# nilsfriess/MultigridMC

Hardware: AMD Instinct MI355X
Metric: MGMC V-cycle samples/sec + fine-smoother HBM GB/s, 512³ lattice, 1/2/4/8 GPUs (higher is better)
Workload: dtype f64

## Files before the change

### multigridmc_amd/csrc/mgmc_capi.hip

```cpp
#include "mgmc_internal.hpp"

namespace mgmc_host {
std::mutex g_err_mutex;
std::string g_last_error;
std::atomic<int> g_live_handles{0};
void set_global_error(const std::string& s) {
    std::lock_guard<std::mutex> lock(g_err_mutex);
    g_last_error = s;
}
}

namespace {
constexpr int LDS_POISON_DOUBLES = 80 * 1024 / 8;
__global__ void __launch_bounds__(1024) k_lds_poison() {
    extern __shared__ double lds[];
    const double nan = __builtin_nan("");
    for (int q = threadIdx.x; q < LDS_POISON_DOUBLES; q += blockDim.x) lds[q] = nan;
    __syncthreads();
    if (lds[(threadIdx.x * 7) % LDS_POISON_DOUBLES] == 0.0) asm volatile("" ::: "memory");
}
__global__ void __launch_bounds__(256) k_poison_interior(Layout L, double* __restrict__ x) {
    const int i = blockIdx.x * blockDim.x + threadIdx.x + 1;
    const int j = blockIdx.y + 1;
    const int k = L.dim == 3 ? (int)blockIdx.z + 1 : 0;
// ... 91 lines not shown
    }
    const int dim = lv.spec.dim, np = lv.spec.npoints;
#define DISPATCH(D, P)                                                       \
    if (dim == D && np == P) {                                               \
        if (noise)                                                           \
            launch_sweep_t<D, P, true>(lv, x, f, g, direction, s);           \
        else                                                                 \
            launch_sweep_t<D, P, false>(lv, x, f, g, direction, s);          \
        return;                                                              \
    }
    DISPATCH(3, 7) DISPATCH(3, 27) DISPATCH(2, 5) DISPATCH(2, 9)
#undef DISPATCH
}

template <int XP, int TY, int NT, int MINW = 1>
void launch_zsweep_t(const Level& lv, ZSweepArgs a, bool prolong, hipStream_t s, int nch) {
    a.ntx = (lv.L.nx / 2) / XP;
    a.nty = (lv.L.ny - 1 + TY - 1) / TY;
    a.ntz = (lv.L.nz - 1 + a.tz - 1) / a.tz;
    const int ntiles = a.ntx * a.nty * (a.zpairs ? (a.ntz + 1) / 2 * 2 : a.ntz);
    const int nb = (ntiles + 7) / 8 * 8;
    const size_t lds = zsweep_lds_bytes(XP, TY, prolong);
    int ex;
    const bool pow2 = std::isnormal(a.alpha) && std::frexp(std::fabs(a.alpha), &ex) == 0.5 && ex > -900 && ex < 900;
    const dim3 grid(nb, 1, nch);
    const bool lrf = a.lr.e != nullptr;
    if (prolong && pow2 && lrf)
        hipLaunchKernelGGL((k_zsweep_rb7<XP, TY, NT, 2, MINW, true>), grid, dim3(NT), lds, s, a);
    else if (prolong && pow2)
        hipLaunchKernelGGL((k_zsweep_rb7<XP, TY, NT, 2, MINW>), grid, dim3(NT), lds, s, a);
    else if (prolong && lrf)
        hipLaunchKernelGGL((k_zsweep_rb7<XP, TY, NT, 1, MINW, true>), grid, dim3(NT), lds, s, a);
    else if (prolong)
        hipLaunchKernelGGL((k_zsweep_rb7<XP, TY, NT, 1, MINW>), grid, dim3(NT), lds, s, a);
    else if (lrf)
        hipLaunchKernelGGL((k_zsweep_rb7<XP, TY, NT, 0, MINW, true>), grid, dim3(NT), lds, s, a);
    else
        hipLaunchKernelGGL((k_zsweep_rb7<XP, TY, NT, 0, MINW>), grid, dim3(NT), lds, s, a);
}

static int zsweep_depth(const Level& lv, int ty, int tzmax) {
// ... 3 lines not shown
    return tz;
}

static int zsweep_plain_rows(const Level& lv, int nch) {
    const int tz = zsweep_depth(lv, ZS_TY, ZS_TZ);
    auto ntiles = [&](int ty) {
        const long long nz = (lv.L.nz - 1 + tz - 1) / tz;
        return (long long)((lv.L.nx / 2) / ZS_XP) * ((lv.L.ny - 1 + ty - 1) / ty) * ((nz + 1) / 2 * 2) * nch;
    };
    const long long slots = 2LL * lv.num_cu;
    return (ZS_TYP != ZS_TY && ZS_NTP == ZS_NT && ntiles(ZS_TY) < slots && ntiles(ZS_TYP) <= slots) ? ZS_TYP : ZS_TY;
}

void launch_zsweep(const Level& lv, const double* xin, double* xout, const double* f, const GibbsArg& g0,
                   int direction, const Level* coarse, const double* xc, double alpha, hipStream_t s, int nch = 1,
                   const LRRhsArg* lr = nullptr) {
    ZSweepArgs a;
    a.lr = lr ? *lr : LRRhsArg{nullptr};
    a.cs = lv.L.nstore;
    a.csc = coarse ? coarse->L.nstore : 0;
    a.L = lv.L;
    a.xin = xin;
    a.xout = xout;
    a.f = f;
    a.xc = xc;
    a.Lc = coarse ? coarse->L : lv.L;
    a.alpha = alpha;
    a.S = lv.S;
    a.G = g0;
    a.G.colour = (direction == MGMC_FORWARD) ? 0 : 1;
    a.zpairs = 0;
    if (coarse) {
        a.tz = zsweep_depth(lv, ZS_TYP, ZS_TZP);
        launch_zsweep_t<ZS_XP, ZS_TYP, ZS_NTP, ZS_MINWP>(lv, a, true, s, nch);
        return;
    }
    a.tz = zsweep_depth(lv, ZS_TY, ZS_TZ);
    a.zpairs = 1;
    if (zsweep_plain_rows(lv, nch) != ZS_TY) {
        launch_zsweep_t<ZS_XP, ZS_TYP, ZS_NTP, ZS_MINWP>(lv, a, false, s, nch);
        return;
    }
    launch_zsweep_t<ZS_XP, ZS_TY, ZS_NT, ZS_MINW>(lv, a, false, s, nch);
}

bool pairs_eligible(const LevelSpec& sp, const Layout& L) {
    return (sp.npoints == 27 || sp.npoints == 9) && L.nx / 2 >= 1 && L.nx / 2 <= 256 && L.nx % 2 == 0;
}

bool quads_eligible(const LevelSpec& sp, const Layout& L, uint32_t paths) {
    if (!pairs_eligible(sp, L) || (paths & PATH_NO_QUADS)) return false;
    return sp.dim == 2 || L.nx / 2 <= tune::QUADS_MAXPAIR;
}

void launch_rb2d(const Level& lv, const double* xin, double* xout, const double* f, const GibbsArg& g, int direction,
                 bool noise, hipStream_t s, int nch = 1) {
    const int ntx = (lv.L.nx - 1 + RB2_TW - 1) / RB2_TW, nty = (lv.L.ny - 1 + RB2_TH - 1) / RB2_TH;
    const int c1 = direction == MGMC_FORWARD ? 0 : 1;
// ... 191 lines not shown
        else if (pre)                                                                                              \
            hipLaunchKernelGGL((k_coarse_ssor_lds<D, P, true>), grid, block, lds, s, lv.L, lv.x, lv.f, lv.S, g,   \
                               nsweeps, nc, chs, nullptr, 0);                                                      \
        else                                                                                                       \
            hipLaunchKernelGGL((k_coarse_ssor_lds<D, P, false>), grid, block, lds, s, lv.L, lv.x, lv.f, lv.S, g,  \
                               nsweeps, nc, chs, nullptr, 0);                                                      \
    } while (0)
    if (dim == 3 && np == 27) MGMC_COARSE_LAUNCH(3, 27);
    else if (dim == 3 && np == 7) MGMC_COARSE_LAUNCH(3, 7);
    else if (dim == 2 && np == 9) MGMC_COARSE_LAUNCH(2, 9);
    else MGMC_COARSE_LAUNCH(2, 5);
#undef MGMC_COARSE_LAUNCH
}


template <int NPTS, int CX, int CY, int NT, bool SYM = false, bool LRF = false>
void launch_zresrestrict_t(const Level& lf, const Level& lc, const double* x, const double* f, double* fc, double* xc,
                           hipStream_t s, int nch, const TailNoiseLaunch* tn = nullptr, const LRRhsArg* lr = nullptr,
                           const PreNoiseLaunch* pn = nullptr) {
    ZRestrictArgs a;
    memset(&a, 0, sizeof(a));
    if (LRF) a.lr = *lr;
    if (pn) {
        a.pn = pn->job;
        a.key = pn->key;
        a.sample = pn->sample;
    }
    a.csf = lf.L.nstore;
    a.csc = lc.L.nstore;
    a.Lf = lf.L;
    a.Lc = lc.L;
// ... 18 lines not shown
        const long long slots = per_cu * lf.num_cu;
        const long long per_chunk = (long long)a.ntx * a.nty;
        long long best = -1;
        for (int kz = 2; kz <= 16; ++kz) {
            const long long tiles = per_chunk * ((lc.L.nz - 1 + kz - 1) / kz);
            const long long cost = ((tiles + slots - 1) / slots) * (2 * kz + 2);
            if (best < 0 || cost < best) {
                best = cost;
                a.kz = kz;
            }
        }
    }
    a.ntz = (lc.L.nz - 1 + a.kz - 1) / a.kz;
    const int nt = a.ntx * a.nty * a.ntz;
    const int nb = (nt + 7) / 8 * 8;
    if (tn && !LRF) {
        a.nblk_main = nb;
        a.jobs = tn->jobs;
        a.njobs = tn->njobs;
        a.zb = tn->zb;
        a.zbs = tn->zbs;
        a.key = tn->key;
        a.chain0 = tn->chain0;
        a.seed_hi = tn->seed_hi;
        a.sample = tn->sample;
        const int nextra = (int)std::min<long long>((tn->zbs + NT - 1) / NT, 64);
        hipLaunchKernelGGL((k_zresrestrict<NPTS, CX, CY, NT, true, SYM>), dim3(nb + nextra, 1, nch), dim3(NT),
                           zrestrict_lds_bytes(CX, CY), s, a);
        return;
    }
    hipLaunchKernelGGL((k_zresrestrict<NPTS, CX, CY, NT, false, SYM, LRF>), dim3(nb, 1, nch), dim3(NT),
                       zrestrict_lds_bytes(CX, CY), s, a);
}

bool zres_lrf_capable(const Level& lf, const Level& lc) {
    return lf.spec.dim == 3 && lf.spec.npoints == 7 && !lf.field && !(lf.paths & PATH_NO_ZRESTRICT) &&
           lc.L.nx >= 8 && lc.L.nx >= tune::ZR_SMALL_NX;
}

bool zres_draws_noise(const Level& lf, const Level& lc) {
    return lf.spec.dim == 3 && lf.spec.npoints == 27 && !lf.field && !(lf.paths & PATH_NO_ZRESTRICT) &&
           lc.L.nx >= tune::ZR_SMALL_NX;
}

void launch_residual_restrict(const Level& lf, const Level& lc, const double* x, const double* f, double* fc,
                              double* xc, int zero_xc, hipStream_t s, int nch, const TailNoiseLaunch* tn,
                              bool skip_xc, const LRRhsArg* lr, const PreNoiseLaunch* pn) {
    const bool zr = lf.spec.dim == 3 && zero_xc && !lf.field && !(lf.paths & PATH_NO_ZRESTRICT) && lc.L.nx >= 8;
    if (nch > 1 && !zr) {
        for (int c = 0; c < nch; ++c)
            launch_residual_restrict(lf, lc, chain_ptr(x, lf, c), chain_ptr(f, lf, c), chain_ptr(fc, lc, c),
                                     chain_ptr(xc, lc, c), zero_xc, s, 1);
        return;
    }
    if (lf.field) {
        dim3 block(64, 4, 1);
        dim3 grid = grid3(lf.L.nx - 1, lf.L.ny - 1, lf.spec.dim == 3 ? lf.L.nz - 1 : 1, block);
        dim3 gc = grid3(lc.L.nx - 1, lc.L.ny - 1, lf.spec.dim == 3 ? lc.L.nz - 1 : 1, block);
        if (lf.spec.dim == 3) {
            hipLaunchKernelGGL((k_fresidual<3>), grid, block, 0, s, lf.L, x, f, lf.F, lf.rbuf);
            hipLaunchKernelGGL((k_restrict<3>), gc, block, 0, s, lf.L, lc.L, (const double*)lf.rbuf, fc);
        } else {
            hipLaunchKernelGGL((k_fresidual<2>), grid, block, 0, s, lf.L, x, f, lf.F, lf.rbuf);
            hipLaunchKernelGGL((k_restrict<2>), gc, block, 0, s, lf.L, lc.L, (const double*)lf.rbuf, fc);
        }
        if (zero_xc) hipMemsetAsync(xc, 0, lc.L.nstore * sizeof(double), s);
        return;
    }
    if (lf.spec.dim == 3 && zero_xc && !(lf.paths & PATH_NO_ZRESTRICT) && lc.L.nx >= 8) {
        const bool small = lc.L.nx < tune::ZR_SMALL_NX;
        if (skip_xc) xc = nullptr;
        if (lr) {
            if ((long long)((lc.L.nx + 62) / 64) * ((lc.L.ny + 6) / 8) * (lc.L.nz - 1) >= tune::ZR7_WIDE_MIN_TILES)
                launch_zresrestrict_t<7, 64, 8, 512, false, true>(lf, lc, x, f, fc, xc, s, nch, nullptr, lr);
            else launch_zresrestrict_t<7, 64, 4, 256, false, true>(lf, lc, x, f, fc, xc, s, nch, nullptr, lr);
        } else if (lf.spec.npoints == 7) {
            if (small) launch_zresrestrict_t<7, 16, 4, 64>(lf, lc, x, f, fc, xc, s, nch, tn);
            else if ((long long)((lc.L.nx + 62) / 64) * ((lc.L.ny + 6) / 8) * (lc.L.nz - 1) >= tune::ZR7_WIDE_MIN_TILES)
                launch_zresrestrict_t<7, 64, 8, 512>(lf, lc, x, f, fc, xc, s, nch);
            else launch_zresrestrict_t<7, 64, 4, 256>(lf, lc, x, f, fc, xc, s, nch);
        } else {
            if (small && lf.fold) launch_zresrestrict_t<27, 16, 4, 64, true>(lf, lc, x, f, fc, xc, s, nch, tn);
            else if (small) launch_zresrestrict_t<27, 16, 4, 64>(lf, lc, x, f, fc, xc, s, nch, tn);
            else if (lf.fold)
                launch_zresrestrict_t<27, tune::ZR27_CX, tune::ZR27_CY, 256, true>(lf, lc, x, f, fc, xc, s, nch, nullptr,
                                                                                   nullptr, pn);
            else launch_zresrestrict_t<27, 64, 4, 256>(lf, lc, x, f, fc, xc, s, nch, nullptr, nullptr, pn);
        }
        return;
    }
// ... 835 lines not shown
        Op& rr = h->ops[q];
        Op& sw = h->ops[q + 1];
        if (rr.kind != OP_RESIDUAL_RESTRICT || sw.kind != OP_SWEEP || sw.level != rr.level + 1 || sw.src != 0 ||
            rr.zpre != 0)
            continue;
        const Level& lf = h->levels[rr.level];
        const Level& lc = h->levels[sw.level];
        const bool zr = lf.spec.dim == 3 && !lf.field && !(lf.paths & PATH_NO_ZRESTRICT) && lc.L.nx >= 8;
        const bool quads3 = lc.quads && lc.spec.dim == 3;
        if (!zr || !(lc.jsweep || quads3) || lc.field) continue;
        rr.xzero = 1;
        sw.xzero = 1;
    }
}

constexpr long long PN_MAX_PAIRS = 2LL << 20;

int plan_drawn_noise(mgmc_handle* h) {
    for (Op& op : h->ops) {
        op.pnz = nullptr;
        op.pn_dst = nullptr;
        op.pn_tag = 0;
    }
    if ((h->paths & PATH_NO_POST_NOISE) || h->nchains != 1) return MGMC_OK;
    std::vector<double2*> buf(h->levels.size(), nullptr);
    auto level_buf = [&](int l) -> double2* {
        if (!buf[l]) {
            const Level& lv = h->levels[l];
            const long long n = (long long)(lv.L.nx / 2) * (lv.L.ny - 1) * (lv.L.nz - 1);
            if (hipMalloc(&buf[l], (size_t)n * sizeof(double2)) != hipSuccess) {
// ... 51 lines not shown
            continue;
        }
        TailArgs* d = h->tail_args[ti];
        const int npn = (int)jobs.size();
        HIPCHK(h, hipMemcpy(d->pn, jobs.data(), jobs.size() * sizeof(PostNoiseJob), hipMemcpyHostToDevice));
        HIPCHK(h, hipMemcpy(&d->npn, &npn, sizeof(int), hipMemcpyHostToDevice));
        h->tail_pn_wg[ti] = tune::TAIL_PN_WG > 0 ? tune::TAIL_PN_WG : std::max(1, h->levels[0].num_cu - h->nchains);
    }
    return MGMC_OK;
}

int build_tails(mgmc_handle* h) {
    int rc = build_tails_only(h);
    if (rc == MGMC_OK) fuse_sweep_restrict(h);
    if (rc == MGMC_OK) mark_zero_inputs(h);
    if (rc == MGMC_OK) rc = plan_drawn_noise(h);
    return rc;
}

void enqueue_ops(mgmc_handle* h, size_t begin, size_t end, hipStream_t s) {
    const uint64_t* sample = h->ctrl;
    const int nch = h->nchains;
    for (size_t q = begin; q < end; ++q) {
        const Op& op = h->ops[q];
        Level& lv = h->levels[op.level];
        if (h->poison)
            hipLaunchKernelGGL(k_lds_poison, dim3(8 * lv.num_cu), dim3(1024), LDS_POISON_DOUBLES * sizeof(double), s);
        switch (op.kind) {
            case OP_SWEEP: {
                GibbsArg g = make_gibbs(h, lv, op.tag, 0, sample);
                const bool lr = lv.lr.m > 0;
                double* fs = lv.f;
                LRRhsArg lrr{nullptr};
                const bool inplace = lr && lv.lr.rhs_inplace;
                if (lr && !op.lr_skip_patch)
                    fs = lr_rhs(h, lv, LR_PATCH_NOISE, lv.f, op.tag, sample, s, nch, -1, inplace ? &lrr : nullptr);
                else if (inplace)
                    lrr = LRRhsArg{lv.lr.rhs_e + nch};
                else if (lr && lv.lr.dense_path)
                    fs = lv.lr.fe2;
                double* xo = lv.x;
                if (lv.zsweep) {
                    const Level* lc = op.prolong ? &h->levels[op.level + 1] : nullptr;
                    xo = lv.buf(1 - op.src);
                    launch_zsweep(lv, lv.buf(op.src), xo, fs, g, op.direction, lc, lc ? lc->x : nullptr,
                                  h->cfg.coarse_scaling, s, nch, lrr.e ? &lrr : nullptr);
                } else if (lv.quads) {
                    xo = lv.buf(1 - op.src);
                    launch_quads(lv, lv.buf(op.src), xo, fs, g, op.direction, s, nch, op.xzero != 0, op.pnz);
                } else if (lv.rb2d) {
                    xo = lv.buf(1 - op.src);
                    launch_rb2d(lv, lv.buf(op.src), xo, fs, g, op.direction, true, s, nch);
                } else if (lv.pairs) {
                    launch_pairs(lv, lv.x, fs, g, op.direction, s, nch);
                } else {
                    launch_sweep(lv, lv.x, fs, g, op.direction, true, s, nch);
                }
                if (lr && lv.lr.small)
                    lr_small(h, lv, xo, op.direction, op.lr_next, op.lr_next_tag, sample, s, nch);
                else if (lr)
                    lr_fix(lv, xo, op.direction, lv.lr.dense_path && !inplace ? nullptr : lv.f, s, nch);
// ... 34 lines not shown
                                lv.lr.rhs_inplace && op.zpre == 0 ? &lrr : nullptr);
                }
                if (op.zpre > 0) {
                    const int ti = op.zpre - 1;
                    const TailNoiseLaunch tn{h->tail_jobs[ti], h->tail_njobs[ti], h->tail_zb[ti], h->tail_zn[ti],
                                             h->key, (uint32_t)h->chain, (uint32_t)(h->seed >> 32), sample};
                    launch_residual_restrict(lv, lc, lv.buf(op.src), fr, lc.f, lc.x, 1, s, nch, &tn);
                } else {
                    PreNoiseLaunch pnl;
                    if (op.pn_dst) {
                        pnl.job = PostNoiseJob{lc.L.nx, lc.L.ny, lc.L.nz, op.pn_tag, op.pn_dst};
                        pnl.key = h->key;
                        pnl.sample = sample;
                    }
                    launch_residual_restrict(lv, lc, lv.buf(op.src), fr, lc.f, lc.x, 1, s, nch, nullptr, op.xzero != 0,
                                             lrr.e ? &lrr : nullptr, op.pn_dst ? &pnl : nullptr);
                    if (op.xzero && h->poison)
                        for (int c = 0; c < nch; ++c)
                            hipLaunchKernelGGL(k_poison_interior, dim3((lc.L.nx - 1 + 255) / 256, lc.L.ny - 1,
                                                                       lc.spec.dim == 3 ? lc.L.nz - 1 : 1),
                                               dim3(256), 0, s, lc.L, chain_ptr(lc.x, lc, c));
                }
                if (lr && lv.lr.dense_path && !lrr.e)
                    ;
                else if (lr && (op.lr_post_patch || op.lr_coarse_patch))
                    lr_restore_patch(h, op, lv, lc, sample, s, nch);
                else if (lr)
                    lr_restore(lv, lv.f, s, nch, lrr.e != nullptr);
                break;
            }
            case OP_PROLONGATE: {
// ... 746 lines not shown

        } else res = "k_residual_restrict<" + std::to_string(dim) + "," + std::to_string(np) + ">";
    }
    std::string text = "sweep=" + sweep;
    if (!post.empty()) text += ";post_sweep=" + post;
    bool by_rr = false, by_tail = false;
    for (size_t q = 0; q < h->ops.size(); ++q) {
        const Op& op = h->ops[q];
        if (op.kind != OP_SWEEP || op.level != level || !op.pnz) continue;
        if (q > 0 && h->ops[q - 1].kind == OP_RESIDUAL_RESTRICT && h->ops[q - 1].pn_dst == op.pnz) by_rr = true;
        else by_tail = true;
    }
    if (by_rr || by_tail)
        text += std::string(";noise=") + (by_rr && by_tail ? "restriction+tail" : by_rr ? "restriction" : "tail");
    if (!res.empty()) text += ";residual_restrict=" + res;
    if (lv.lr.m > 0)
        text += std::string(";lowrank=") + (lv.lr.rhs_inplace ? "dense,rhs_inplace" : lv.lr.dense_path ? "dense"
                                             : lv.lr.small ? "small" : "rows");
    snprintf(out, n, "%s", text.c_str());
    return MGMC_OK;
}

static int put_fine(mgmc_handle* h, double* v, int c, const double* host, size_t n, const char* what) {
    if (!h || !host) return fail(h, MGMC_E_INVALID, "null argument");
    if (n != h->levels[0].spec.ndof) return fail(h, MGMC_E_INVALID, std::string(what) + " size mismatch");
    if (c >= h->nchains) return fail(h, MGMC_E_INVALID, "chain index out of range");
    HIPCHK(h, hipSetDevice(h->device));
    const size_t ns = h->levels[0].L.nstore;
    int rc = upload(h, 0, host, v + (size_t)std::max(c, 0) * ns);
    if (rc) return rc;
    if (c < 0)
        for (int q = 1; q < h->nchains; ++q)
            HIPCHK(h, hipMemcpyAsync(v + q * ns, v, ns * sizeof(double), hipMemcpyDeviceToDevice, h->stream));
    return MGMC_OK;
}

int mgmc_set_rhs(mgmc_handle* h, const double* f, size_t n) {
    int rc = put_fine(h, h ? h->levels[0].f : nullptr, -1, f, n, "rhs");
    if (rc) return rc;
    HIPCHK(h, hipStreamSynchronize(h->stream));
    return MGMC_OK;
}

static int set_state_impl(mgmc_handle* h, int c, const double* x, size_t n) {
    int rc = put_fine(h, h ? h->levels[0].x : nullptr, c, x, n, "state");
    if (rc) return rc;
    HIPCHK(h, hipMemsetAsync(h->ctrl + 5, 0, sizeof(uint64_t), h->stream));
    HIPCHK(h, hipStreamSynchronize(h->stream));
    return MGMC_OK;
}

int mgmc_set_state(mgmc_handle* h, const double* x, size_t n) { return set_state_impl(h, -1, x, n); }

int mgmc_set_state_chain(mgmc_handle* h, int chain, const double* x, size_t n) {
    if (chain < 0) return fail(h, MGMC_E_INVALID, "chain index out of range");
// ... 484 lines not shown
```

### multigridmc_amd/csrc/mgmc_internal.hpp

```cpp
#pragma once
#include <hip/hip_runtime.h>
#include <rccl/rccl.h>
#include <stdio.h>
#include <stdlib.h>
#include <string.h>

#include <algorithm>
#include <atomic>
#include <cmath>
#include <mutex>
#include <string>
#include <vector>

#include "../../include/mgmc.h"
#include "mgmc_hierarchy.hpp"
#include "mgmc_kernels.hpp"
#include "mgmc_zsweep.hpp"
#include "mgmc_tuning.hpp"
#include "mgmc_layout_check.hpp"
static_assert(MGMC_LAYOUT_POINT == mgmc::LF_POINT && MGMC_LAYOUT_PAIRS == mgmc::LF_PAIRS &&
                  MGMC_LAYOUT_ZSWEEP == mgmc::LF_ZSWEEP && MGMC_LAYOUT_ZSWEEP_COARSE == mgmc::LF_ZSWEEP_C &&
                  MGMC_LAYOUT_ZRESTRICT == mgmc::LF_ZRESTRICT && MGMC_LAYOUT_RB2D == mgmc::LF_RB2D &&
                  MGMC_LAYOUT_JSWEEP == mgmc::LF_JSWEEP && MGMC_LAYOUT_QRESTRICT == mgmc::LF_QRESTRICT,
              "layout family bits");
#include "mgmc_zrestrict.hpp"
#include "mgmc_tail.hpp"
#include "mgmc_gsweep.hpp"
#include "mgmc_qrestrict.hpp"
#include "mgmc_jsweep.hpp"
#include "mgmc_rb2d.hpp"
#include "mgmc_lowrank.hpp"
#include "mgmc_solver.hpp"
#include "mgmc_cholesky.hpp"
#include "mgmc_field.hpp"
#include "mgmc_operators.hpp"

using namespace mgmc;

namespace mgmc_host {

void set_global_error(const std::string& s);

enum OpKind {
    OP_SWEEP = 0,
    OP_RESIDUAL_RESTRICT = 1,
    OP_PROLONGATE = 2,
    OP_COARSE_LDS = 3,
    OP_QOI = 4,
    OP_COPY = 5,
    OP_COARSE_CHOL = 6,
// ... 6 lines not shown
    int level;
    int direction;
    uint32_t tag;
    int nsweeps;
    int src = 0;
    int prolong = 0;
    int lr_next = 0;
    uint32_t lr_next_tag = 0;
    int lr_skip_patch = 0;
    int lr_post_patch = 0;
    uint32_t lr_post_tag = 0;
    int lr_coarse_patch = 0;
    uint32_t lr_coarse_tag = 0;
    int tail = -1;
    int xzero = 0;
    int zpre = 0;
    const double2* pnz = nullptr;
    double2* pn_dst = nullptr;
    uint32_t pn_tag = 0;
};


enum PathFlag : uint32_t {
    PATH_NO_TAIL = 1u << 0,
    PATH_NO_FUSE_PROLONG = 1u << 1,
    PATH_NO_QUADS = 1u << 2,
    PATH_NO_RB2D = 1u << 3,
    PATH_NO_ZSWEEP = 1u << 4,
    PATH_NO_PAIRS = 1u << 5,
    PATH_NO_ZRESTRICT = 1u << 6,
// ... 144 lines not shown

}

using namespace mgmc_host;

struct mgmc_handle {
    LiveHandleCount live;
    mgmc_config cfg;
    int device = 0;
    uint64_t seed = 0, chain = 0;
    int nchains = 1;
    RngKey key;
    std::vector<Level> levels;
    hipStream_t stream = nullptr;
    uint64_t* ctrl = nullptr;
    double* mom = nullptr;
    double* series = nullptr;
    uint64_t series_cap = 0;
    double* lex_tmp = nullptr;
    size_t lex_cap = 0;
    std::vector<Op> ops;
    size_t seg_end_pre = 0, seg_begin_post = 0, seg_end_post = 0;
    hipGraphExec_t graph_all = nullptr;
    hipGraphExec_t graph_unroll = nullptr;
    hipGraph_t graph_timed_src = nullptr;
    hipGraphExec_t graph_timed = nullptr;
    hipGraphNode_t timed_node[5] = {nullptr, nullptr, nullptr, nullptr, nullptr};
    hipEvent_t timed_ev0[5] = {nullptr, nullptr, nullptr, nullptr, nullptr};
    int unroll = 1;
    int64_t qoi_store_index = -1;
// ... 72 lines not shown
struct PreNoiseLaunch {
    PostNoiseJob job;
    RngKey key;
    const uint64_t* sample;
};
enum LRScale { LR_SCALE_ONE = 0, LR_SCALE_INV = 1 };

namespace mgmc_host {
dim3 grid3(int nthreads_x, int nrows_y, int nz_blocks, dim3 block);
GibbsArg make_gibbs(const mgmc_handle* h, const Level& lv, uint32_t tag, int colour, const uint64_t* sample);
void launch_sweep(const Level& lv, double* x, const double* f, const GibbsArg& g0, int direction, bool noise,
                  hipStream_t s, int nch = 1);
bool zres_lrf_capable(const Level& lf, const Level& lc);
void launch_residual_restrict(const Level& lf, const Level& lc, const double* x, const double* f, double* fc,
                              double* xc, int zero_xc, hipStream_t s, int nch = 1, const TailNoiseLaunch* tn = nullptr,
                              bool skip_xc = false, const LRRhsArg* lr = nullptr, const PreNoiseLaunch* pn = nullptr);
bool zres_draws_noise(const Level& lf, const Level& lc);
void launch_prolongate(const Level& lf, const Level& lc, double* x, const double* xc, double alpha, hipStream_t s,
                       int nch = 1);
void lr_dots(const Level& lv, const double* v, LRScale scale, hipStream_t s, int nch = 1);
double* lr_rhs(const mgmc_handle* h, const Level& lv, int mode, double* f, uint32_t tag, const uint64_t* sample,
               hipStream_t s, int nch = 1, int64_t post_tag = -1, LRRhsArg* inplace = nullptr);
void lr_fix(const Level& lv, double* x, int direction, double* f_restore, hipStream_t s, int nch = 1);
void lr_restore(const Level& lv, double* f, hipStream_t s, int nch = 1, bool patched = false);
void launch_operator_apply(const mgmc_handle* h, const Level& lv, const double* xs, double* ys, hipStream_t s);
void launch_coarse_chol(const mgmc_handle* h, const Level& lv, const double* f, double* x, bool noise, uint32_t tag,
                        const uint64_t* sample, hipStream_t s, int nch = 1);
Layout tail_layout(const Layout& L);
void build_ops(mgmc_handle* h);
int build_tails(mgmc_handle* h);
int build_graphs(mgmc_handle* h);
void destroy_graphs(mgmc_handle* h);
int ensure_scratch(mgmc_handle* h, int level);
int upload(mgmc_handle* h, int level, const double* host, double* pad);
int download(mgmc_handle* h, int level, const double* pad, double* host);
int refuse_unusable(mgmc_handle* h);
int check_level(mgmc_handle* h, int level, bool need_coarser);
int build_coarse_chol(mgmc_handle* h, const std::vector<LRColumn>* cols, const double* sigma, int m);
}
```

### multigridmc_amd/csrc/mgmc_kernels.hpp

```cpp
#pragma once
#include <hip/hip_runtime.h>
#include <stdint.h>

#include "philox_normal.h"

namespace mgmc {

struct Layout {
    int dim;
    int nx, ny, nz;
    int off;
    int pad_;
    long long sx, sp, nstore;
    __host__ __device__ long long at(int i, int j, int k) const {
        return (long long)k * sp + (long long)j * sx + (long long)i + off;
    }
};

inline Layout make_layout(int dim, const int n[3], bool reach2 = false) {
    Layout L;
    L.dim = dim;
    L.nx = n[0];
    L.ny = n[1];
    L.nz = dim == 3 ? n[2] : 0;
// ... 621 lines not shown
        *reinterpret_cast<double2*>(x + p) = v;
    }
}

template <int DIM, int NPTS>
__global__ void __launch_bounds__(256) k_operator_apply(Layout L, const double* __restrict__ x, double* __restrict__ y,
                                                        StencilArg S) {
    const int i = blockIdx.x * blockDim.x + threadIdx.x + 1;
    const int j = blockIdx.y * blockDim.y + threadIdx.y + 1;
    const int k = (DIM == 3) ? (int)blockIdx.z + 1 : 0;
    if (i > L.nx - 1 || j > L.ny - 1) return;
    const long long p = L.at(i, j, k);
    y[p] = stencil_sum<DIM, NPTS>(x, p, L, S);
}

template <int DIM>
__global__ void __launch_bounds__(256) k_pack(Layout L, const double* __restrict__ lex, double* __restrict__ pad) {
    const int i = blockIdx.x * blockDim.x + threadIdx.x + 1;
    const int j = blockIdx.y * blockDim.y + threadIdx.y + 1;
    const int k = (DIM == 3) ? (int)blockIdx.z + 1 : 0;
    if (i > L.nx - 1 || j > L.ny - 1) return;
    const long long row = (DIM == 3) ? (long long)(k - 1) * (L.ny - 1) + (j - 1) : (long long)(j - 1);
    pad[L.at(i, j, k)] = lex[row * (L.nx - 1) + (i - 1)];
}

template <int DIM>
__global__ void __launch_bounds__(256) k_unpack(Layout L, const double* __restrict__ pad, double* __restrict__ lex) {
    const int i = blockIdx.x * blockDim.x + threadIdx.x + 1;
    const int j = blockIdx.y * blockDim.y + threadIdx.y + 1;
    const int k = (DIM == 3) ? (int)blockIdx.z + 1 : 0;
// ... 117 lines not shown
```

### multigridmc_amd/csrc/mgmc_zrestrict.hpp

```cpp
#pragma once
#include "mgmc_kernels.hpp"
#include "mgmc_tail.hpp"
#include "mgmc_tuning.hpp"
#include <type_traits>

namespace mgmc {

struct ZRestrictArgs {
    Layout Lf, Lc;
    const double* x;
    const double* f;
    double* fc;
    double* xc;
    StencilArg S;
    int kz;
    int ntx, nty, ntz;
    long long csf, csc;
    int nblk_main;
    const TailNoiseJob* jobs;
    int njobs;
    double2* zb;
    long long zbs;
    RngKey key;
    uint32_t chain0, seed_hi;
// ... 5 lines not shown
#define ZR_RD(n, o) "ds_read_b64 %" #n ", %12 offset:" #o "\n"
template <int RB, int EV>
__device__ __forceinline__ void zr_plane12(uint32_t base, double (&v)[12]) {
    static_assert(2 * RB + EV < 65536 && EV >= 8, "ds offsets");
    asm volatile(ZR_RD(0, 0) ZR_RD(1, 8) ZR_RD(2, %c13) ZR_RD(3, %c14)
                 ZR_RD(4, %c15) ZR_RD(5, %c16) ZR_RD(6, %c17) ZR_RD(7, %c18)
                 ZR_RD(8, %c19) ZR_RD(9, %c20) ZR_RD(10, %c21) ZR_RD(11, %c22) "s_waitcnt lgkmcnt(0)"
                 : "=&v"(v[0]), "=&v"(v[1]), "=&v"(v[2]), "=&v"(v[3]), "=&v"(v[4]), "=&v"(v[5]), "=&v"(v[6]),
                   "=&v"(v[7]), "=&v"(v[8]), "=&v"(v[9]), "=&v"(v[10]), "=&v"(v[11])
                 : "v"(base), "i"(EV - 8), "i"(EV), "i"(RB), "i"(RB + 8), "i"(RB + EV - 8), "i"(RB + EV),
                   "i"(2 * RB), "i"(2 * RB + 8), "i"(2 * RB + EV - 8), "i"(2 * RB + EV)
                 : "memory");
}
#undef ZR_RD

template <int NPTS, int CX, int CY, int NT, bool ZN = false, bool SYM = false, bool LRF = false>
__global__ void __launch_bounds__(NT) __attribute__((amdgpu_waves_per_eu(NPTS == 27 && SYM && CX >= 48 ? tune::ZR27_MINW : 1)))
k_zresrestrict(ZRestrictArgs a) {
    if (ZN && (int)blockIdx.x >= a.nblk_main) {
        const int ch = batch_chain();
        RngKey key = a.key;
        if (ch) key.k1 = (a.chain0 + (uint32_t)ch) ^ a.seed_hi;
        const uint64_t sample = *a.sample;
        double2* z = a.zb + ch * a.zbs;
        const int nw = ((int)gridDim.x - a.nblk_main) * NT;
        const int w0 = ((int)blockIdx.x - a.nblk_main) * NT + (int)threadIdx.x;
        for (int jb = 0; jb < a.njobs; ++jb) {
            const TailNoiseJob J = a.jobs[jb];
            const int npair = J.nx / 2, nyi = J.ny - 1;
            const int n = npair * nyi * (J.nz - 1);
            for (int q = w0; q < n; q += nw) {
                const int m = q % npair, row = q / npair;
                const int i0 = 2 * m + 1;
// ... 14 lines not shown
    constexpr int RSr = 2 * RP + 2;
    constexpr int XPP = CX + 3;
    constexpr int XR = 2 * CY + 3;
    constexpr int XS = 2 * XPP + 2;
    constexpr int XPS = XR * XS;
    constexpr int NLX = (XR * XPP + NT - 1) / NT;
    constexpr int NLR = (RR * RP + NT - 1) / NT;
    constexpr int NCP = (CX * CY + NT - 1) / NT;
    extern __shared__ __attribute__((aligned(16))) double smem[];
    double* xs = smem;
    double* rs = xs + 3 * XPS;

    {
        const int ch = batch_chain();
        a.x += ch * a.csf;
        a.f += ch * a.csf;
        a.fc += ch * a.csc;
        a.xc += ch * a.csc;
        if (LRF) a.lr.e += ch;
    }
    const double lre = LRF ? *a.lr.e : 0.0;
    const Layout& Lf = a.Lf;
    const Layout& Lc = a.Lc;
    const int nb = ZN ? a.nblk_main : (int)gridDim.x, b = blockIdx.x, per = nb >> 3;
    const int tile = (nb & 7) ? b : (b & 7) * per + (b >> 3);
    const int txi = tile % a.ntx;
    const int tyi = (tile / a.ntx) % a.nty;
    const int tzi = tile / (a.ntx * a.nty);
    auto draw_pn = [&]() {
        if (!a.pn.dst) return;
        const uint64_t sample = *a.sample;
// ... 70 lines not shown
    auto issue_x = [&](int k) {
        const double* base = plane_ptr(a.x, k > kx_last ? kx_last : k);
#pragma unroll
        for (int u = 0; u < NLX; ++u) px[u] = *reinterpret_cast<const double2*>(base + xoff[u]);
    };
    auto deposit_x = [&](int k) {
        double* dst = xs + xslot(k) * XPS;
#pragma unroll
        for (int u = 0; u < NLX; ++u)
            if (xlds[u] >= 0) {
                dst[xlds[u]] = px[u].x;
                dst[xlds[u] + XPP] = px[u].y;
            }
    };
    auto issue_f = [&](int k) {
        const double* base = plane_ptr(a.f, k > kf_last ? kf_last : k);
#pragma unroll
        for (int u = 0; u < NLR; ++u) pf[u] = *reinterpret_cast<const double2*>(base + roff[u]);
    };
    auto residual = [&](int k, const double2 (&fv)[NLR]) {
        const bool kin = k >= 1 && k <= Lf.nz - 1;
        const double* pl[3] = {xs + xslot(k - 1) * XPS, xs + xslot(k) * XPS, xs + xslot(k + 1) * XPS};
#pragma unroll
        for (int u = 0; u < NLR; ++u) {
            if (rlds[u] < 0) continue;
            const int o0 = rxo[u], o1 = rxo[u] + XPP;
            const int m0 = o0 + XPP - 1, m1 = o1 - XPP;
            double y0 = 0.0, y1 = 0.0;
            if (NPTS == 7) {
                y0 += a.S.a[4] * pl[0][o0];
// ... 34 lines not shown
                for (int dz = 0; dz < 3; ++dz) {
                    double v[12];
                    zr_plane12<XS * 8, XPP * 8>(lds_addr(pl[dz] - XS + o0), v);
#pragma unroll
                    for (int r = 0; r < 3; ++r) {
                        const int c = dz * 9 + r * 3;
                        y0 += a.S.a[c] * v[4 * r + 2];
                        y1 += a.S.a[c] * v[4 * r + 0];
                        y0 += a.S.a[c + 1] * v[4 * r + 0];
                        y1 += a.S.a[c + 1] * v[4 * r + 3];
                        y0 += a.S.a[c + 2] * v[4 * r + 3];
                        y1 += a.S.a[c + 2] * v[4 * r + 1];
                    }
                }
            }
            double2 f = fv[u];
            if constexpr (LRF) f = lr_rhs_pair(f, lre);
            rs[rlds[u]] = (kin && (rflag[u] & 1)) ? f.x - y0 : 0.0;
            rs[rlds[u] + RP] = (kin && (rflag[u] & 2)) ? f.y - y1 : 0.0;
        }
    };
    auto accumulate = [&](double (&acc)[NCP], int sz) {
#pragma unroll
        for (int u = 0; u < NCP; ++u) {
            double result = acc[u];
#pragma unroll
            for (int sy = -1; sy <= 1; ++sy)
#pragma unroll
                for (int sx = -1; sx <= 1; ++sx) {
                    double w = 1.0;
                    w *= w1(sx);
// ... 58 lines not shown
```

### multigridmc_amd/csrc/mgmc_zsweep.hpp

```cpp
#pragma once
#include <type_traits>

#include "mgmc_kernels.hpp"
#include "mgmc_tuning.hpp"

namespace mgmc {

struct ZSweepArgs {
    Layout L;
    const double* xin;
    double* xout;
    const double* f;
    const double* xc;
    Layout Lc;
    double alpha;
    StencilArg S;
    GibbsArg G;
    int tz;
    int ntx, nty, ntz;
    int zpairs;
    long long cs, csc;
    LRRhsArg lr;
};

struct ZItem {
    int goff;
    uint32_t pbase;
    int lds;
    int flags;
};

struct RunE0 {
    int value;
};

constexpr int zs_threads(int TY) { return 256 * ((TY / 2 + 2 + 3) / 4); }

template <int XP, int TY, int NT, int PROLONG, int MINW, bool LRF = false>
__global__ void __launch_bounds__(NT) __attribute__((amdgpu_waves_per_eu(MINW))) k_zsweep_rb7(ZSweepArgs a) {
    static_assert(XP == 32 && TY % 4 == 0 && TY <= 32 && NT == zs_threads(TY), "tile shape");
    constexpr int WP = XP + 2;
    constexpr int RS = 2 * WP + 2;
    constexpr int R = TY + 4;
    constexpr int PS = R * RS;
    constexpr int NSLOT = 4;
    constexpr int NCW = TY / 2;
    constexpr int NLX = (R * WP + NT - 1) / NT;
    extern __shared__ __attribute__((aligned(16))) double smem[];
    double* xs = smem;
    double* tab = xs + NSLOT * PS;
    for (int q = threadIdx.x; q < 64; q += NT) {
        tab[q] = LOGTAB_RC[q];
        tab[64 + q] = LOGTAB_HI[q];
        tab[128 + q] = LOGTAB_LO[q];
    }
    for (int q = threadIdx.x; q < 130; q += NT) tab[192 + q] = SINCOS_TAB[q];
    if (!PROLONG) __syncthreads();
    constexpr int CW = XP + 8, CWP = CW / 2, CR = TY / 2 + 3, CPS = CR * CW;
    constexpr int NLC = PROLONG ? (CR * CWP + NT - 1) / NT : 1;
    double* cring = tab + 322;

    {
        const int ch = batch_chain();
        a.xin += ch * a.cs;
        a.xout += ch * a.cs;
        a.f += ch * a.cs;
        if (PROLONG) a.xc += ch * a.csc;
        a.G.key = chain_key(a.G, ch);
        if (LRF) a.lr.e += ch;
    }
    const double lre = LRF ? *a.lr.e : 0.0;
    const Layout& L = a.L;
    const int nb = gridDim.x;
    const int b = blockIdx.x;
    const int per = nb >> 3;
    const int tile = (nb & 7) ? b : (b & 7) * per + (b >> 3);
    int txi = tile % a.ntx;
    int tyi = (tile / a.ntx) % a.nty;
    int tzi = tile / (a.ntx * a.nty);
    bool down = false;
    if (!PROLONG && a.zpairs) {
// ... 208 lines not shown
            constexpr bool odd_step = decltype(ODDc)::value;
            const int e = odd_step ? 1 - E0c_v : E0c_v;
            const int o1 = t.lds + e * WP, o2 = t.lds + (1 - e) * WP;
            const bool inf = e ? in1 : in0;
            using Bp = std::integral_constant<int, odd_step ? 0 : 1>;
            deposit_x(p + dz, std::integral_constant<int, DN ? -1 : (odd_step ? 0 : 1)>{}, Bp{});
            if (PROLONG) {
                if (odd_step) deposit_c((p + 3) / 2);
                else issue_c((p + 4) / 2);
            }
            if constexpr (PF2) {
                issue_x(p + 3, Bp{});
                (void)fnxt;
            } else {
                issue_x(p + 2 * dz, Bp{});
                if (active_wave) fnxt = load_f(p + dz);
            }
            __syncthreads();
            if (interior_plane(p) && active_wave) {
                double2 fv = fcur;
                if constexpr (LRF) fv = lr_rhs_pair(fv, lre);
                if (inf) {
                    const double res = row_sum(p, o1, e, xs[slot(p - 1) * PS + o1]);
                    const double crhs = fma(sd, e ? z.y : z.x, e ? fv.y : fv.x);
                    double* s0 = xs + slot(p) * PS;
                    s0[o1] = fma(wd, crhs - res, s0[o1]);
                }
                pk_out = fma(sd, e ? z.x : z.y, e ? fv.x : fv.y);
            }
            if constexpr (PF2) fcur = load_f(p + 2);
            __syncthreads();
            const int k = p - dz;
            if (core_wave) {
                const bool own = k >= k0 && k < k1;
                const double* s0 = xs + slot(k) * PS;
                const double fv = s0[o2];
                if (own && rowin) {
                    double sv = s0[o1];
                    if (inf) {
                        const double res = DN ? row_sum_ba(k, o1, e, xs[slot(p) * PS + o1], fb) : row_sum(k, o1, e, fb);
                        sv = fma(wd, pk_in - res, sv);
                    }
                    double* dst = a.xout + (long long)k * L.sp + t.goff;
                    const double2 out = e ? make_double2(fv, sv) : make_double2(sv, fv);
                    __builtin_nontemporal_store(out.x, dst);
                    __builtin_nontemporal_store(out.y, dst + 1);
                }
                fb = fv;
            }
            if (active_wave && interior_plane(p + dz)) z = noise(p + dz);
        };
        double2 fA = make_double2(0.0, 0.0), fB = make_double2(0.0, 0.0);
        double pkA = 0.0, pkB = 0.0;
        const int pst = DN ? k1 : k0 - 1;
        if constexpr (PF2) {
            fA = load_f(k0 - 1);
            fB = load_f(k0);
        } else if (active_wave) {
            fA = load_f(pst);
        }
        if (active_wave && interior_plane(pst)) z = noise(pst);
        if constexpr (DN) {
            for (int p = k1; p >= k0 - 1; p -= 2) {
                step(p, std::integral_constant<bool, false>{}, fA, fB, pkB, pkA);
                if (p - 1 >= k0 - 1) step(p - 1, std::integral_constant<bool, true>{}, fB, fA, pkA, pkB);
            }
        } else {
            for (int p = k0 - 1; p <= k1; p += 2) {
                step(p, std::integral_constant<bool, false>{}, fA, fB, pkB, pkA);
                if (p + 1 <= k1) step(p + 1, std::integral_constant<bool, true>{}, fB, fA, pkA, pkB);
// ... 52 lines not shown
```

Measured before the change: 422.8.

## Skip right-hand-side loads in fine smoother and restriction when RHS is zero

Adds a device OR-reduction over the fine right-hand side when it is set, and records whether it is identically zero. When it is, the fine-level z-sweep and 7-point residual-restrict kernels are instantiated with a flag that never reads f and treats it as zero, and the graphs are rebuilt. This removes one full-grid stream of HBM reads per sweep and restriction. The cost is an extra reduction kernel and host sync in set_rhs, plus more kernel instantiations.

```diff
diff --git a/multigridmc_amd/csrc/mgmc_capi.hip b/multigridmc_amd/csrc/mgmc_capi.hip
--- a/multigridmc_amd/csrc/mgmc_capi.hip
+++ b/multigridmc_amd/csrc/mgmc_capi.hip
@@ -129,7 +129,7 @@
 }
 
 template <int XP, int TY, int NT, int MINW = 1>
-void launch_zsweep_t(const Level& lv, ZSweepArgs a, bool prolong, hipStream_t s, int nch) {
+void launch_zsweep_t(const Level& lv, ZSweepArgs a, bool prolong, hipStream_t s, int nch, bool fz) {
     a.ntx = (lv.L.nx / 2) / XP;
     a.nty = (lv.L.ny - 1 + TY - 1) / TY;
     a.ntz = (lv.L.nz - 1 + a.tz - 1) / a.tz;
@@ -140,6 +140,15 @@
     const bool pow2 = std::isnormal(a.alpha) && std::frexp(std::fabs(a.alpha), &ex) == 0.5 && ex > -900 && ex < 900;
     const dim3 grid(nb, 1, nch);
     const bool lrf = a.lr.e != nullptr;
+    if (fz && !lrf) {
+        if (prolong && pow2)
+            hipLaunchKernelGGL((k_zsweep_rb7<XP, TY, NT, 2, MINW, false, true>), grid, dim3(NT), lds, s, a);
+        else if (prolong)
+            hipLaunchKernelGGL((k_zsweep_rb7<XP, TY, NT, 1, MINW, false, true>), grid, dim3(NT), lds, s, a);
+        else
+            hipLaunchKernelGGL((k_zsweep_rb7<XP, TY, NT, 0, MINW, false, true>), grid, dim3(NT), lds, s, a);
+        return;
+    }
     if (prolong && pow2 && lrf)
         hipLaunchKernelGGL((k_zsweep_rb7<XP, TY, NT, 2, MINW, true>), grid, dim3(NT), lds, s, a);
     else if (prolong && pow2)
@@ -173,7 +182,7 @@
 
 void launch_zsweep(const Level& lv, const double* xin, double* xout, const double* f, const GibbsArg& g0,
                    int direction, const Level* coarse, const double* xc, double alpha, hipStream_t s, int nch = 1,
-                   const LRRhsArg* lr = nullptr) {
+                   const LRRhsArg* lr = nullptr, bool fzero = false) {
     ZSweepArgs a;
     a.lr = lr ? *lr : LRRhsArg{nullptr};
     a.cs = lv.L.nstore;
@@ -191,16 +200,16 @@
     a.zpairs = 0;
     if (coarse) {
         a.tz = zsweep_depth(lv, ZS_TYP, ZS_TZP);
-        launch_zsweep_t<ZS_XP, ZS_TYP, ZS_NTP, ZS_MINWP>(lv, a, true, s, nch);
+        launch_zsweep_t<ZS_XP, ZS_TYP, ZS_NTP, ZS_MINWP>(lv, a, true, s, nch, fzero);
         return;
     }
     a.tz = zsweep_depth(lv, ZS_TY, ZS_TZ);
     a.zpairs = 1;
     if (zsweep_plain_rows(lv, nch) != ZS_TY) {
-        launch_zsweep_t<ZS_XP, ZS_TYP, ZS_NTP, ZS_MINWP>(lv, a, false, s, nch);
+        launch_zsweep_t<ZS_XP, ZS_TYP, ZS_NTP, ZS_MINWP>(lv, a, false, s, nch, fzero);
         return;
     }
-    launch_zsweep_t<ZS_XP, ZS_TY, ZS_NT, ZS_MINW>(lv, a, false, s, nch);
+    launch_zsweep_t<ZS_XP, ZS_TY, ZS_NT, ZS_MINW>(lv, a, false, s, nch, fzero);
 }
 
 bool pairs_eligible(const LevelSpec& sp, const Layout& L) {
@@ -422,7 +431,7 @@
 }
 
 
-template <int NPTS, int CX, int CY, int NT, bool SYM = false, bool LRF = false>
+template <int NPTS, int CX, int CY, int NT, bool SYM = false, bool LRF = false, bool FZ = false>
 void launch_zresrestrict_t(const Level& lf, const Level& lc, const double* x, const double* f, double* fc, double* xc,
                            hipStream_t s, int nch, const TailNoiseLaunch* tn = nullptr, const LRRhsArg* lr = nullptr,
                            const PreNoiseLaunch* pn = nullptr) {
@@ -471,7 +480,7 @@
     a.ntz = (lc.L.nz - 1 + a.kz - 1) / a.kz;
     const int nt = a.ntx * a.nty * a.ntz;
     const int nb = (nt + 7) / 8 * 8;
-    if (tn && !LRF) {
+    if (tn && !LRF && !FZ) {
         a.nblk_main = nb;
         a.jobs = tn->jobs;
         a.njobs = tn->njobs;
@@ -486,7 +495,7 @@
                            zrestrict_lds_bytes(CX, CY), s, a);
         return;
     }
-    hipLaunchKernelGGL((k_zresrestrict<NPTS, CX, CY, NT, false, SYM, LRF>), dim3(nb, 1, nch), dim3(NT),
+    hipLaunchKernelGGL((k_zresrestrict<NPTS, CX, CY, NT, false, SYM, LRF, FZ>), dim3(nb, 1, nch), dim3(NT),
                        zrestrict_lds_bytes(CX, CY), s, a);
 }
 
@@ -502,7 +511,7 @@
 
 void launch_residual_restrict(const Level& lf, const Level& lc, const double* x, const double* f, double* fc,
                               double* xc, int zero_xc, hipStream_t s, int nch, const TailNoiseLaunch* tn,
-                              bool skip_xc, const LRRhsArg* lr, const PreNoiseLaunch* pn) {
+                              bool skip_xc, const LRRhsArg* lr, const PreNoiseLaunch* pn, bool fzero) {
     const bool zr = lf.spec.dim == 3 && zero_xc && !lf.field && !(lf.paths & PATH_NO_ZRESTRICT) && lc.L.nx >= 8;
     if (nch > 1 && !zr) {
         for (int c = 0; c < nch; ++c)
@@ -531,6 +540,10 @@
             if ((long long)((lc.L.nx + 62) / 64) * ((lc.L.ny + 6) / 8) * (lc.L.nz - 1) >= tune::ZR7_WIDE_MIN_TILES)
                 launch_zresrestrict_t<7, 64, 8, 512, false, true>(lf, lc, x, f, fc, xc, s, nch, nullptr, lr);
             else launch_zresrestrict_t<7, 64, 4, 256, false, true>(lf, lc, x, f, fc, xc, s, nch, nullptr, lr);
+        } else if (lf.spec.npoints == 7 && fzero && !small) {
+            if ((long long)((lc.L.nx + 62) / 64) * ((lc.L.ny + 6) / 8) * (lc.L.nz - 1) >= tune::ZR7_WIDE_MIN_TILES)
+                launch_zresrestrict_t<7, 64, 8, 512, false, false, true>(lf, lc, x, f, fc, xc, s, nch);
+            else launch_zresrestrict_t<7, 64, 4, 256, false, false, true>(lf, lc, x, f, fc, xc, s, nch);
         } else if (lf.spec.npoints == 7) {
             if (small) launch_zresrestrict_t<7, 16, 4, 64>(lf, lc, x, f, fc, xc, s, nch, tn);
             else if ((long long)((lc.L.nx + 62) / 64) * ((lc.L.ny + 6) / 8) * (lc.L.nz - 1) >= tune::ZR7_WIDE_MIN_TILES)
@@ -1396,6 +1409,25 @@
     }
 }
 
+static RhsZeroOp rhs_zero_op(const mgmc_handle* h, const Op& op) {
+    const Level& lv = h->levels[op.level];
+    const bool has_coarse = op.level + 1 < (int)h->levels.size();
+    return RhsZeroOp{op.level, lv.zsweep, lv.lr.m, lv.spec.npoints, !(lv.paths & PATH_NO_ZRESTRICT),
+                     has_coarse ? h->levels[op.level + 1].L.nx : 0, tune::ZR_SMALL_NX, op.zpre};
+}
+bool mark_rhs_zero(mgmc_handle* h) {
+    bool changed = false;
+    for (Op& op : h->ops) {
+        const int z = (op.kind == OP_SWEEP && rhs_zero_sweep_ok(h->f0_zero, rhs_zero_op(h, op))) ||
+                              (op.kind == OP_RESIDUAL_RESTRICT && rhs_zero_residual_ok(h->f0_zero, rhs_zero_op(h, op)))
+                          ? 1
+                          : 0;
+        changed = changed || z != op.fzero;
+        op.fzero = z;
+    }
+    return changed;
+}
+
 constexpr long long PN_MAX_PAIRS = 2LL << 20;
 
 int plan_drawn_noise(mgmc_handle* h) {
@@ -1477,6 +1509,7 @@
     int rc = build_tails_only(h);
     if (rc == MGMC_OK) fuse_sweep_restrict(h);
     if (rc == MGMC_OK) mark_zero_inputs(h);
+    if (rc == MGMC_OK) mark_rhs_zero(h);
     if (rc == MGMC_OK) rc = plan_drawn_noise(h);
     return rc;
 }
@@ -1507,7 +1540,7 @@
                     const Level* lc = op.prolong ? &h->levels[op.level + 1] : nullptr;
                     xo = lv.buf(1 - op.src);
                     launch_zsweep(lv, lv.buf(op.src), xo, fs, g, op.direction, lc, lc ? lc->x : nullptr,
-                                  h->cfg.coarse_scaling, s, nch, lrr.e ? &lrr : nullptr);
+                                  h->cfg.coarse_scaling, s, nch, lrr.e ? &lrr : nullptr, op.fzero != 0);
                 } else if (lv.quads) {
                     xo = lv.buf(1 - op.src);
                     launch_quads(lv, lv.buf(op.src), xo, fs, g, op.direction, s, nch, op.xzero != 0, op.pnz);
@@ -1572,7 +1605,7 @@
                         pnl.sample = sample;
                     }
                     launch_residual_restrict(lv, lc, lv.buf(op.src), fr, lc.f, lc.x, 1, s, nch, nullptr, op.xzero != 0,
-                                             lrr.e ? &lrr : nullptr, op.pn_dst ? &pnl : nullptr);
+                                             lrr.e ? &lrr : nullptr, op.pn_dst ? &pnl : nullptr, op.fzero != 0);
                     if (op.xzero && h->poison)
                         for (int c = 0; c < nch; ++c)
                             hipLaunchKernelGGL(k_poison_interior, dim3((lc.L.nx - 1 + 255) / 256, lc.L.ny - 1,
@@ -2349,6 +2382,11 @@
     if (by_rr || by_tail)
         text += std::string(";noise=") + (by_rr && by_tail ? "restriction+tail" : by_rr ? "restriction" : "tail");
     if (!res.empty()) text += ";residual_restrict=" + res;
+    for (const Op& op : h->ops)
+        if (op.level == level && op.fzero) {
+            text += ";rhs=zero";
+            break;
+        }
     if (lv.lr.m > 0)
         text += std::string(";lowrank=") + (lv.lr.rhs_inplace ? "dense,rhs_inplace" : lv.lr.dense_path ? "dense"
                                              : lv.lr.small ? "small" : "rows");
@@ -2373,7 +2411,20 @@
 int mgmc_set_rhs(mgmc_handle* h, const double* f, size_t n) {
     int rc = put_fine(h, h ? h->levels[0].f : nullptr, -1, f, n, "rhs");
     if (rc) return rc;
+    unsigned long long bits = 0;
+    unsigned long long* word = reinterpret_cast<unsigned long long*>(h->ctrl + 7);
+    HIPCHK(h, hipMemsetAsync(word, 0, sizeof(*word), h->stream));
+    const int nblk = (int)std::min<size_t>((n + 255) / 256, (size_t)16 * h->levels[0].num_cu);
+    hipLaunchKernelGGL(k_or_bits, dim3(nblk), dim3(256), 0, h->stream,
+                       reinterpret_cast<const unsigned long long*>(h->lex_tmp), (long long)n, word);
+    HIPCHK(h, hipGetLastError());
+    HIPCHK(h, hipMemcpyAsync(&bits, word, sizeof(bits), hipMemcpyDeviceToHost, h->stream));
     HIPCHK(h, hipStreamSynchronize(h->stream));
+    const bool zero = rhs_bits_all_zero(bits);
+    if (zero != h->f0_zero) {
+        h->f0_zero = zero;
+        if (mark_rhs_zero(h)) return build_graphs(h);
+    }
     return MGMC_OK;
 }
 
diff --git a/multigridmc_amd/csrc/mgmc_internal.hpp b/multigridmc_amd/csrc/mgmc_internal.hpp
--- a/multigridmc_amd/csrc/mgmc_internal.hpp
+++ b/multigridmc_amd/csrc/mgmc_internal.hpp
@@ -34,6 +34,7 @@
 #include "mgmc_cholesky.hpp"
 #include "mgmc_field.hpp"
 #include "mgmc_operators.hpp"
+#include "mgmc_rhs_zero.hpp"
 
 using namespace mgmc;
 
@@ -70,6 +71,7 @@
     uint32_t lr_coarse_tag = 0;
     int tail = -1;
     int xzero = 0;
+    int fzero = 0;
     int zpre = 0;
     const double2* pnz = nullptr;
     double2* pn_dst = nullptr;
@@ -244,6 +246,7 @@
     std::vector<Level> levels;
     hipStream_t stream = nullptr;
     uint64_t* ctrl = nullptr;
+    bool f0_zero = true;
     double* mom = nullptr;
     double* series = nullptr;
     uint64_t series_cap = 0;
@@ -346,7 +349,8 @@
 bool zres_lrf_capable(const Level& lf, const Level& lc);
 void launch_residual_restrict(const Level& lf, const Level& lc, const double* x, const double* f, double* fc,
                               double* xc, int zero_xc, hipStream_t s, int nch = 1, const TailNoiseLaunch* tn = nullptr,
-                              bool skip_xc = false, const LRRhsArg* lr = nullptr, const PreNoiseLaunch* pn = nullptr);
+                              bool skip_xc = false, const LRRhsArg* lr = nullptr, const PreNoiseLaunch* pn = nullptr,
+                              bool fzero = false);
 bool zres_draws_noise(const Level& lf, const Level& lc);
 void launch_prolongate(const Level& lf, const Level& lc, double* x, const double* xc, double alpha, hipStream_t s,
                        int nch = 1);
@@ -361,6 +365,7 @@
 Layout tail_layout(const Layout& L);
 void build_ops(mgmc_handle* h);
 int build_tails(mgmc_handle* h);
+bool mark_rhs_zero(mgmc_handle* h);
 int build_graphs(mgmc_handle* h);
 void destroy_graphs(mgmc_handle* h);
 int ensure_scratch(mgmc_handle* h, int level);
diff --git a/multigridmc_amd/csrc/mgmc_kernels.hpp b/multigridmc_amd/csrc/mgmc_kernels.hpp
--- a/multigridmc_amd/csrc/mgmc_kernels.hpp
+++ b/multigridmc_amd/csrc/mgmc_kernels.hpp
@@ -659,6 +659,15 @@
     y[p] = stencil_sum<DIM, NPTS>(x, p, L, S);
 }
 
+static __global__ void __launch_bounds__(256) k_or_bits(const unsigned long long* __restrict__ v, long long n,
+                                                 unsigned long long* __restrict__ out) {
+    unsigned long long acc = 0;
+    const long long stride = (long long)gridDim.x * 256;
+    for (long long q = (long long)blockIdx.x * 256 + threadIdx.x; q < n; q += stride) acc |= v[q];
+    for (int o = 32; o > 0; o >>= 1) acc |= __shfl_xor(acc, o);
+    if ((threadIdx.x & 63) == 0 && acc) atomicOr(out, acc);
+}
+
 template <int DIM>
 __global__ void __launch_bounds__(256) k_pack(Layout L, const double* __restrict__ lex, double* __restrict__ pad) {
     const int i = blockIdx.x * blockDim.x + threadIdx.x + 1;
diff --git a/multigridmc_amd/csrc/mgmc_rhs_zero.hpp b/multigridmc_amd/csrc/mgmc_rhs_zero.hpp
--- /dev/null
+++ b/multigridmc_amd/csrc/mgmc_rhs_zero.hpp
@@ -0,0 +1,40 @@
+#pragma once
+#include <cstddef>
+#include <cstdint>
+#include <cstring>
+
+namespace mgmc_host {
+
+inline bool rhs_bits_all_zero(uint64_t or_bits) { return or_bits == 0; }
+
+inline uint64_t rhs_or_bits(const double* v, size_t n) {
+    uint64_t acc = 0;
+    for (size_t q = 0; q < n; ++q) {
+        uint64_t b;
+        std::memcpy(&b, v + q, sizeof(b));
+        acc |= b;
+    }
+    return acc;
+}
+
+struct RhsZeroOp {
+    int level;
+    bool zsweep;
+    int lr_m;
+    int npoints;
+    bool zrestrict;
+    int coarse_nx;
+    int small_nx;
+    int zpre;
+};
+
+inline bool rhs_zero_sweep_ok(bool f0_zero, const RhsZeroOp& o) {
+    return f0_zero && o.level == 0 && o.zsweep && o.lr_m == 0;
+}
+
+inline bool rhs_zero_residual_ok(bool f0_zero, const RhsZeroOp& o) {
+    return f0_zero && o.level == 0 && o.zsweep && o.lr_m == 0 && o.npoints == 7 && o.zrestrict && o.zpre == 0 &&
+           o.coarse_nx >= 8 && o.coarse_nx >= o.small_nx;
+}
+
+}
diff --git a/multigridmc_amd/csrc/mgmc_zrestrict.hpp b/multigridmc_amd/csrc/mgmc_zrestrict.hpp
--- a/multigridmc_amd/csrc/mgmc_zrestrict.hpp
+++ b/multigridmc_amd/csrc/mgmc_zrestrict.hpp
@@ -43,9 +43,10 @@
 }
 #undef ZR_RD
 
-template <int NPTS, int CX, int CY, int NT, bool ZN = false, bool SYM = false, bool LRF = false>
+template <int NPTS, int CX, int CY, int NT, bool ZN = false, bool SYM = false, bool LRF = false, bool FZ = false>
 __global__ void __launch_bounds__(NT) __attribute__((amdgpu_waves_per_eu(NPTS == 27 && SYM && CX >= 48 ? tune::ZR27_MINW : 1)))
 k_zresrestrict(ZRestrictArgs a) {
+    static_assert(!(LRF && FZ), "a patched right-hand side is not zero");
     if (ZN && (int)blockIdx.x >= a.nblk_main) {
         const int ch = batch_chain();
         RngKey key = a.key;
@@ -90,7 +91,7 @@
     {
         const int ch = batch_chain();
         a.x += ch * a.csf;
-        a.f += ch * a.csf;
+        if (!FZ) a.f += ch * a.csf;
         a.fc += ch * a.csc;
         a.xc += ch * a.csc;
         if (LRF) a.lr.e += ch;
@@ -191,6 +192,7 @@
             }
     };
     auto issue_f = [&](int k) {
+        if constexpr (FZ) return;
         const double* base = plane_ptr(a.f, k > kf_last ? kf_last : k);
 #pragma unroll
         for (int u = 0; u < NLR; ++u) pf[u] = *reinterpret_cast<const double2*>(base + roff[u]);
@@ -255,7 +257,8 @@
                     }
                 }
             }
-            double2 f = fv[u];
+            double2 f = make_double2(0.0, 0.0);
+            if constexpr (!FZ) f = fv[u];
             if constexpr (LRF) f = lr_rhs_pair(f, lre);
             rs[rlds[u]] = (kin && (rflag[u] & 1)) ? f.x - y0 : 0.0;
             rs[rlds[u] + RP] = (kin && (rflag[u] & 2)) ? f.y - y1 : 0.0;
diff --git a/multigridmc_amd/csrc/mgmc_zsweep.hpp b/multigridmc_amd/csrc/mgmc_zsweep.hpp
--- a/multigridmc_amd/csrc/mgmc_zsweep.hpp
+++ b/multigridmc_amd/csrc/mgmc_zsweep.hpp
@@ -36,9 +36,10 @@
 
 constexpr int zs_threads(int TY) { return 256 * ((TY / 2 + 2 + 3) / 4); }
 
-template <int XP, int TY, int NT, int PROLONG, int MINW, bool LRF = false>
+template <int XP, int TY, int NT, int PROLONG, int MINW, bool LRF = false, bool FZ = false>
 __global__ void __launch_bounds__(NT) __attribute__((amdgpu_waves_per_eu(MINW))) k_zsweep_rb7(ZSweepArgs a) {
     static_assert(XP == 32 && TY % 4 == 0 && TY <= 32 && NT == zs_threads(TY), "tile shape");
+    static_assert(!(LRF && FZ), "a patched right-hand side is not zero");
     constexpr int WP = XP + 2;
     constexpr int RS = 2 * WP + 2;
     constexpr int R = TY + 4;
@@ -64,7 +65,7 @@
         const int ch = batch_chain();
         a.xin += ch * a.cs;
         a.xout += ch * a.cs;
-        a.f += ch * a.cs;
+        if (!FZ) a.f += ch * a.cs;
         if (PROLONG) a.xc += ch * a.csc;
         a.G.key = chain_key(a.G, ch);
         if (LRF) a.lr.e += ch;
@@ -303,11 +304,14 @@
                 (void)fnxt;
             } else {
                 issue_x(p + 2 * dz, Bp{});
-                if (active_wave) fnxt = load_f(p + dz);
+                if constexpr (!FZ) {
+                    if (active_wave) fnxt = load_f(p + dz);
+                }
             }
             __syncthreads();
             if (interior_plane(p) && active_wave) {
-                double2 fv = fcur;
+                double2 fv = make_double2(0.0, 0.0);
+                if constexpr (!FZ) fv = fcur;
                 if constexpr (LRF) fv = lr_rhs_pair(fv, lre);
                 if (inf) {
                     const double res = row_sum(p, o1, e, xs[slot(p - 1) * PS + o1]);
@@ -317,7 +321,7 @@
                 }
                 pk_out = fma(sd, e ? z.x : z.y, e ? fv.x : fv.y);
             }
-            if constexpr (PF2) fcur = load_f(p + 2);
+            if constexpr (PF2 && !FZ) fcur = load_f(p + 2);
             __syncthreads();
             const int k = p - dz;
             if (core_wave) {
@@ -342,7 +346,8 @@
         double2 fA = make_double2(0.0, 0.0), fB = make_double2(0.0, 0.0);
         double pkA = 0.0, pkB = 0.0;
         const int pst = DN ? k1 : k0 - 1;
-        if constexpr (PF2) {
+        if constexpr (FZ) {
+        } else if constexpr (PF2) {
             fA = load_f(k0 - 1);
             fB = load_f(k0);
         } else if (active_wave) {
```

Result: faster. 500.9 (median of 6 runs) (+18.5%).
